# DLR-RM/AugmentedAutoencoder

Hardware: NVIDIA H100
Metric: pose queries/sec (encode+codebook NN) (higher is better)
Workload: dtype f32 via split-fp16 tensor-core products (3x, fp32 accumulate)

## Files before the change

### augmentedautoencoder_b200/csrc/tc_common.cuh

```cuda
#pragma once
#include <cuda.h>
#include <cuda_fp16.h>
#include <cuda_runtime.h>
#include <stdint.h>

namespace aae {
namespace tc {

__device__ __forceinline__ uint32_t smem_u32(const void* p) { return (uint32_t)__cvta_generic_to_shared(p); }

__device__ __forceinline__ bool elect_one() {
  uint32_t pred = 0;
  asm volatile(
      "{\n\t"
      ".reg .pred P1;\n\t"
      "elect.sync _|P1, 0xffffffff;\n\t"
      "selp.b32 %0, 1, 0, P1;\n\t"
      "}\n"
      : "=r"(pred));
  return pred != 0;
}

__device__ __forceinline__ void mbar_init(uint64_t* bar, uint32_t count) {
  asm volatile("mbarrier.init.shared::cta.b64 [%0], %1;" ::"r"(smem_u32(bar)), "r"(count));
}
__device__ __forceinline__ void fence_barrier_init() { asm volatile("fence.mbarrier_init.release.cluster;" ::: "memory"); }
__device__ __forceinline__ void fence_proxy_async_smem() { asm volatile("fence.proxy.async.shared::cta;" ::: "memory"); }

__device__ __forceinline__ void mbar_arrive_expect_tx(uint64_t* bar, uint32_t bytes) {
  asm volatile("mbarrier.arrive.expect_tx.shared::cta.b64 _, [%0], %1;" ::"r"(smem_u32(bar)), "r"(bytes) : "memory");
}
__device__ __forceinline__ void mbar_arrive(uint64_t* bar) {
  asm volatile("mbarrier.arrive.shared::cta.b64 _, [%0];" ::"r"(smem_u32(bar)) : "memory");
}
__device__ __forceinline__ bool mbar_try_wait(uint64_t* bar, uint32_t parity) {
  uint32_t ok;
  asm volatile(
      "{\n\t"
      ".reg .pred P1;\n\t"
      "mbarrier.try_wait.parity.shared::cta.b64 P1, [%1], %2;\n\t"
      "selp.b32 %0, 1, 0, P1;\n\t"
      "}\n"
      : "=r"(ok)
      : "r"(smem_u32(bar)), "r"(parity)
      : "memory");
  return ok != 0;
}
__device__ __forceinline__ void mbar_wait(uint64_t* bar, uint32_t parity) {
  while (!mbar_try_wait(bar, parity)) {
  }
}

__device__ __forceinline__ void prefetch_tmap(const CUtensorMap* m) {
  asm volatile("prefetch.tensormap [%0];" ::"l"(reinterpret_cast<uint64_t>(m)) : "memory");
}
__device__ __forceinline__ void tma_load_2d(void* smem_dst, const CUtensorMap* m, uint64_t* bar, int c0, int c1) {
  asm volatile("cp.async.bulk.tensor.2d.shared::cluster.global.mbarrier::complete_tx::bytes [%0], [%1, {%3, %4}], [%2];" ::"r"(
                   smem_u32(smem_dst)),
               "l"(reinterpret_cast<uint64_t>(m)), "r"(smem_u32(bar)), "r"(c0), "r"(c1)
               : "memory");
}
__device__ __forceinline__ void tma_load_4d(void* smem_dst, const CUtensorMap* m, uint64_t* bar, int c0, int c1, int c2, int c3) {
  asm volatile(
      "cp.async.bulk.tensor.4d.shared::cluster.global.mbarrier::complete_tx::bytes [%0], [%1, {%3, %4, %5, %6}], [%2];" ::"r"(
          smem_u32(smem_dst)),
      "l"(reinterpret_cast<uint64_t>(m)), "r"(smem_u32(bar)), "r"(c0), "r"(c1), "r"(c2), "r"(c3)
      : "memory");
}

__device__ __forceinline__ void bulk_store_1d(void* gmem_dst, const void* smem_src, uint32_t bytes) {
  asm volatile("cp.async.bulk.global.shared::cta.bulk_group [%0], [%1], %2;" ::"l"(gmem_dst), "r"(smem_u32(smem_src)), "r"(bytes) : "memory");
}
__device__ __forceinline__ void bulk_commit_group() { asm volatile("cp.async.bulk.commit_group;" ::: "memory"); }
__device__ __forceinline__ void bulk_wait_read_all() { asm volatile("cp.async.bulk.wait_group.read 0;" ::: "memory"); }
__device__ __forceinline__ void bulk_wait_all() { asm volatile("cp.async.bulk.wait_group 0;" ::: "memory"); }
__device__ __forceinline__ void tma_store_2d(const CUtensorMap* m, const void* smem_src, int c0, int c1) {
  asm volatile("cp.async.bulk.tensor.2d.global.shared::cta.bulk_group [%0, {%2, %3}], [%1];" ::"l"(reinterpret_cast<uint64_t>(m)),
               "r"(smem_u32(smem_src)), "r"(c0), "r"(c1)
               : "memory");
}
__device__ __forceinline__ void tma_store_5d(const CUtensorMap* m, const void* smem_src, int c0, int c1, int c2, int c3, int c4) {
  asm volatile("cp.async.bulk.tensor.5d.global.shared::cta.bulk_group [%0, {%2, %3, %4, %5, %6}], [%1];" ::"l"(reinterpret_cast<uint64_t>(m)),
               "r"(smem_u32(smem_src)), "r"(c0), "r"(c1), "r"(c2), "r"(c3), "r"(c4)
               : "memory");
}

template <int N>
struct Wgmma;
#define AAE_D8(i) "+f"(d[i]), "+f"(d[i + 1]), "+f"(d[i + 2]), "+f"(d[i + 3]), "+f"(d[i + 4]), "+f"(d[i + 5]), "+f"(d[i + 6]), "+f"(d[i + 7])
template <>
struct Wgmma<64> {
  template <int TA, int TB>
  static __device__ __forceinline__ void ss(float (&d)[32], uint64_t da, uint64_t db, uint32_t accumulate) {
    asm volatile(
        "{\n\t.reg .pred p;\n\tsetp.ne.b32 p, %34, 0;\n\t"
        "wgmma.mma_async.sync.aligned.m64n64k16.f32.f16.f16 {%0, %1, %2, %3, %4, %5, %6, %7, %8, %9, %10, %11, %12, %13, %14, %15, %16, %17, %18, %19, %20, %21, %22, %23, %24, %25, %26, %27, %28, %29, %30, %31}, %32, %33, p, 1, 1, %35, %36;\n\t}\n"
        : AAE_D8(0), AAE_D8(8), AAE_D8(16), AAE_D8(24)
        : "l"(da), "l"(db), "r"(accumulate), "n"(TA), "n"(TB));
  }
};

template <>
struct Wgmma<128> {
  template <int TA, int TB>
  static __device__ __forceinline__ void ss(float (&d)[64], uint64_t da, uint64_t db, uint32_t accumulate) {
    asm volatile(
        "{\n\t.reg .pred p;\n\tsetp.ne.b32 p, %66, 0;\n\t"
        "wgmma.mma_async.sync.aligned.m64n128k16.f32.f16.f16 {%0, %1, %2, %3, %4, %5, %6, %7, %8, %9, %10, %11, %12, %13, %14, %15, %16, %17, %18, %19, %20, %21, %22, %23, %24, %25, %26, %27, %28, %29, %30, %31, %32, %33, %34, %35, %36, %37, %38, %39, %40, %41, %42, %43, %44, %45, %46, %47, %48, %49, %50, %51, %52, %53, %54, %55, %56, %57, %58, %59, %60, %61, %62, %63}, %64, %65, p, 1, 1, %67, %68;\n\t}\n"
        : AAE_D8(0), AAE_D8(8), AAE_D8(16), AAE_D8(24), AAE_D8(32), AAE_D8(40), AAE_D8(48), AAE_D8(56)
        : "l"(da), "l"(db), "r"(accumulate), "n"(TA), "n"(TB));
  }
};

__device__ __forceinline__ void wgmma_fence() { asm volatile("wgmma.fence.sync.aligned;" ::: "memory"); }
__device__ __forceinline__ void wgmma_commit() { asm volatile("wgmma.commit_group.sync.aligned;" ::: "memory"); }
template <int N>
__device__ __forceinline__ void wgmma_wait() { asm volatile("wgmma.wait_group.sync.aligned %0;" ::"n"(N) : "memory"); }
template <int R>
__device__ __forceinline__ void wgmma_fence_regs(float (&d)[R]) {
#pragma unroll
  for (int i = 0; i < R; ++i) asm volatile("" : "+f"(d[i])::"memory");
}

__device__ __forceinline__ void cp_async_16(void* smem_dst, const void* gmem_src, bool pred) {
  const int bytes = pred ? 16 : 0;
  asm volatile("cp.async.cg.shared.global [%0], [%1], 16, %2;" ::"r"(smem_u32(smem_dst)), "l"(gmem_src), "r"(bytes) : "memory");
}
__device__ __forceinline__ void cp_async_wait_all() { asm volatile("cp.async.wait_all;" ::: "memory"); }
__device__ __forceinline__ void named_bar_sync(int id, int threads) { asm volatile("bar.sync %0, %1;" ::"r"(id), "r"(threads) : "memory"); }

__device__ __forceinline__ uint64_t make_sw128_kmajor_desc(uint32_t smem_addr) {
  uint64_t d = 0;
  d |= (uint64_t)((smem_addr & 0x3FFFF) >> 4);
  d |= (uint64_t)1 << 16;
  d |= (uint64_t)(1024 >> 4) << 32;
  d |= (uint64_t)1 << 62;
  return d;
}
__device__ __forceinline__ uint64_t make_sw128_mnmajor_desc(uint32_t smem_addr, uint32_t lbo_bytes, uint32_t sbo_bytes) {
  uint64_t d = 0;
  d |= (uint64_t)((smem_addr & 0x3FFFF) >> 4);
  d |= (uint64_t)(lbo_bytes >> 4) << 16;
  d |= (uint64_t)(sbo_bytes >> 4) << 32;
  d |= (uint64_t)1 << 62;
  return d;
}
__device__ __forceinline__ uint64_t desc_advance_k(uint64_t desc, int k_step) { return desc + (uint64_t)((k_step * 32) >> 4); }

__device__ __forceinline__ void split_f16(float x, __half& hi, __half& lo) {
  hi = __float2half_rn(x);
  lo = __float2half_rn(x - __half2float(hi));
}

__device__ __forceinline__ void split_f16x2(float a, float b, uint32_t& hi2, uint32_t& lo2) {
  const float ca = __fmul_rn(a, 8193.0f), cb = __fmul_rn(b, 8193.0f);
  const float ha = __fsub_rn(ca, __fsub_rn(ca, a)), hb = __fsub_rn(cb, __fsub_rn(cb, b));
  const __half2 h = __floats2half2_rn(ha, hb);
  const __half2 l = __floats2half2_rn(__fsub_rn(a, ha), __fsub_rn(b, hb));
  hi2 = *reinterpret_cast<const uint32_t*>(&h);
  lo2 = *reinterpret_cast<const uint32_t*>(&l);
}

}

typedef CUresult (*PFN_tmapEncodeTiled)(CUtensorMap*, CUtensorMapDataType, cuuint32_t, void*, const cuuint64_t*, const cuuint64_t*,
                                        const cuuint32_t*, const cuuint32_t*, CUtensorMapInterleave, CUtensorMapSwizzle,
                                        CUtensorMapL2promotion, CUtensorMapFloatOOBfill);
PFN_tmapEncodeTiled get_tmap_encoder();
int make_tmap_f16(CUtensorMap* out, const void* base, int rank, const uint64_t* dims, const uint64_t* strides_bytes, const uint32_t* box,
                  int swizzle_bytes = 128);

}
```

### augmentedautoencoder_b200/csrc/tc_gemm.cu

```cuda
#include <algorithm>
#include <vector>

#include "tc.cuh"
#include "tc_common.cuh"
#include "tc_plan.cuh"

namespace aae {

using namespace tc;

PFN_tmapEncodeTiled get_tmap_encoder() {
  static PFN_tmapEncodeTiled fn = nullptr;
  if (!fn) {
    void* p = nullptr;
    cudaDriverEntryPointQueryResult q;
    if (cudaGetDriverEntryPoint("cuTensorMapEncodeTiled", &p, cudaEnableDefault, &q) == cudaSuccess && q == cudaDriverEntryPointSuccess)
      fn = reinterpret_cast<PFN_tmapEncodeTiled>(p);
  }
  return fn;
}

int make_tmap_f16(CUtensorMap* out, const void* base, int rank, const uint64_t* dims, const uint64_t* strides_bytes, const uint32_t* box,
                  int swizzle_bytes) {
  PFN_tmapEncodeTiled enc = get_tmap_encoder();
  if (!enc) { set_error("cuTensorMapEncodeTiled is unavailable in this driver"); return AAE_ERR_CUDA; }
  cuuint64_t gdim[5], gstr[4];
  cuuint32_t bx[5], es[5];
  for (int i = 0; i < rank; ++i) { gdim[i] = dims[i]; bx[i] = box[i]; es[i] = 1; }
  for (int i = 0; i + 1 < rank; ++i) gstr[i] = strides_bytes[i];
  CUresult r = enc(out, CU_TENSOR_MAP_DATA_TYPE_FLOAT16, (cuuint32_t)rank, const_cast<void*>(base), gdim, gstr, bx, es,
                   CU_TENSOR_MAP_INTERLEAVE_NONE, swizzle_bytes == 64 ? CU_TENSOR_MAP_SWIZZLE_64B : CU_TENSOR_MAP_SWIZZLE_128B,
                   CU_TENSOR_MAP_L2_PROMOTION_L2_256B,
                   CU_TENSOR_MAP_FLOAT_OOB_FILL_NONE);
  if (r != CUDA_SUCCESS) { set_error("cuTensorMapEncodeTiled failed with CUresult %d (rank %d)", (int)r, rank); return AAE_ERR_CUDA; }
  return AAE_OK;
}

template <int N_TILE, int STAGES, int PLANES = 2>
struct TcSmem {
  static constexpr int A_BYTES = 128 * TC_KCH * 2;
  static constexpr int W_BYTES = N_TILE * TC_KCH * 2;
  static constexpr int STAGE_BYTES = PLANES * A_BYTES + PLANES * W_BYTES;
  static constexpr int ACC_LD = PLANES * N_TILE + 4;
  static constexpr int ACC_BYTES = 128 * ACC_LD * 4;
  static constexpr int BODY = STAGES * STAGE_BYTES > ACC_BYTES ? STAGES * STAGE_BYTES : ACC_BYTES;
  static constexpr int TOTAL = BODY + 1024  + 256 ;
};

template <int N_TILE, int STAGES, int PLANES = 2>
__global__ void __launch_bounds__(TC_THREADS, 1)
tc_gemm_kernel(const __grid_constant__ CUtensorMap tm_a_hi, const __grid_constant__ CUtensorMap tm_a_lo,
               const __grid_constant__ CUtensorMap tm_w_hi, const __grid_constant__ CUtensorMap tm_w_lo, const TcGemmParams p) {
  using S = TcSmem<N_TILE, STAGES, PLANES>;
  constexpr int R = N_TILE / 2;
  extern __shared__ uint8_t smem_raw[];
  uint8_t* smem = reinterpret_cast<uint8_t*>((reinterpret_cast<uintptr_t>(smem_raw) + 1023) & ~(uintptr_t)1023);
  uint64_t* full_bar = reinterpret_cast<uint64_t*>(smem + S::BODY);
  uint64_t* empty_bar = full_bar + STAGES;

  const int warp = threadIdx.x >> 5;
  const int lane = threadIdx.x & 31;
  const int m0 = blockIdx.y * 128;
  const int n0 = blockIdx.x * N_TILE;
  const int total_iters = p.taps * p.chunks_per_tap;
  const int it_begin = blockIdx.z * p.iters_per_split;
  const int it_end = min(total_iters, it_begin + p.iters_per_split);

  if (threadIdx.x == 0) {
    prefetch_tmap(&tm_a_hi);
    if constexpr (PLANES == 2) prefetch_tmap(&tm_a_lo);
    prefetch_tmap(&tm_w_hi);
    if constexpr (PLANES == 2) prefetch_tmap(&tm_w_lo);
    for (int s = 0; s < STAGES; ++s) { mbar_init(&full_bar[s], 1); mbar_init(&empty_bar[s], 2); }
    fence_barrier_init();
  }
  __syncthreads();

  if (warp == 0) {
    if (lane == 0) {
      const int hw = p.OH * p.OW;
      const int b0 = m0 / hw, rem = m0 - b0 * hw;
      const int oh0 = rem / p.OW, ow0 = rem - oh0 * p.OW;
      for (int it = it_begin, i = 0; it < it_end; ++it, ++i) {
        const int s = i % STAGES;
        const uint32_t ph = (uint32_t)(i / STAGES) & 1u;
        mbar_wait(&empty_bar[s], ph ^ 1u);
        const int tap = it / p.chunks_per_tap, cc = it - tap * p.chunks_per_tap;
        uint8_t* st = smem + s * S::STAGE_BYTES;
        mbar_arrive_expect_tx(&full_bar[s], S::STAGE_BYTES);
        const int c0 = p.tap_ch[tap] + cc * TC_KCH;
        const int x = ow0 + p.tap_dj[tap], y = oh0 + p.tap_di[tap];
        const int kcol = it * TC_KCH;
        tma_load_4d(st, &tm_a_hi, &full_bar[s], c0, x, y, b0);
        if constexpr (PLANES == 2) tma_load_4d(st + S::A_BYTES, &tm_a_lo, &full_bar[s], c0, x, y, b0);
        tma_load_2d(st + PLANES * S::A_BYTES, &tm_w_hi, &full_bar[s], kcol, n0);
        if constexpr (PLANES == 2) tma_load_2d(st + 2 * S::A_BYTES + S::W_BYTES, &tm_w_lo, &full_bar[s], kcol, n0);
      }
    }
  } else if (warp >= 4) {
    const int wg = (warp - 4) >> 2;
    float acc[R], crs[R];
#pragma unroll
    for (int j = 0; j < R; ++j) { acc[j] = 0.f; crs[j] = 0.f; }
    for (int it = it_begin, i = 0; it < it_end; ++it, ++i) {
      const int s = i % STAGES;
      mbar_wait(&full_bar[s], (uint32_t)(i / STAGES) & 1u);
      const uint32_t st = smem_u32(smem + s * S::STAGE_BYTES);
      const uint32_t a_off = (uint32_t)(wg * 64 * TC_KCH * 2);
      const uint64_t a_hi = make_sw128_kmajor_desc(st + a_off);
      const uint64_t a_lo = make_sw128_kmajor_desc(st + S::A_BYTES + a_off);
      const uint64_t w_hi = make_sw128_kmajor_desc(st + PLANES * S::A_BYTES);
      const uint64_t w_lo = make_sw128_kmajor_desc(st + 2 * S::A_BYTES + S::W_BYTES);
      wgmma_fence_regs(acc);
      if constexpr (PLANES == 2) wgmma_fence_regs(crs);
      wgmma_fence();
#pragma unroll
      for (int k = 0; k < TC_KCH / 16; ++k) {
        const uint32_t first = (i > 0 || k > 0) ? 1u : 0u;
        Wgmma<N_TILE>::template ss<0, 0>(acc, desc_advance_k(a_hi, k), desc_advance_k(w_hi, k), first);
        if constexpr (PLANES == 2) {
          Wgmma<N_TILE>::template ss<0, 0>(crs, desc_advance_k(a_lo, k), desc_advance_k(w_hi, k), first);
          Wgmma<N_TILE>::template ss<0, 0>(crs, desc_advance_k(a_hi, k), desc_advance_k(w_lo, k), 1u);
        }
      }
      wgmma_commit();
      wgmma_wait<1>();
      wgmma_fence_regs(acc);
      if constexpr (PLANES == 2) wgmma_fence_regs(crs);
      if (i > 0 && (warp & 3) == 0 && lane == 0) mbar_arrive(&empty_bar[(i - 1) % STAGES]);
    }
    wgmma_wait<0>();
    wgmma_fence_regs(acc);
    if constexpr (PLANES == 2) wgmma_fence_regs(crs);
    named_bar_sync(1, 256);
    float* img = reinterpret_cast<float*>(smem);
    tc_park_acc<PLANES>(img, S::ACC_LD, wg, warp, lane, acc, crs);
    named_bar_sync(1, 256);
    tc_epilogue<PLANES, N_TILE>(p, img, S::ACC_LD, m0, n0, it_end > it_begin, warp, lane);
  }
}

namespace {

template <int PLANES>
__global__ void pack_weights_kernel(const float* __restrict__ w, int taps, int cin, int cout, float scale, __half* __restrict__ hi,
                                    __half* __restrict__ lo, unsigned* __restrict__ range_flag, unsigned range_bit) {
  __shared__ float tile[32][33];
  const int tap = blockIdx.z;
  const int ci0 = blockIdx.y * 32, co0 = blockIdx.x * 32;
  for (int i = threadIdx.y; i < 32; i += 8) {
    const int ci = ci0 + i, co = co0 + threadIdx.x;
    tile[i][threadIdx.x] = (ci < cin && co < cout) ? w[((long long)tap * cin + ci) * cout + co] : 0.f;
  }
  __syncthreads();
  for (int i = threadIdx.y; i < 32; i += 8) {
    const int co = co0 + i, ci = ci0 + threadIdx.x;
    if (co < cout && ci < cin)
      tc_store_f16<PLANES>(tile[threadIdx.x][i] * scale, hi, lo, (long long)co * taps * cin + (long long)tap * cin + ci, range_flag, range_bit);
  }
}

template <int PLANES>
__global__ void unpack_act_kernel(const __half* __restrict__ hi, const __half* __restrict__ lo, int B, int H, int W, int C, int s2d,
                                  float inv_scale, float* __restrict__ out) {
  const long long total = (long long)B * H * W * C;
  for (long long i = (long long)blockIdx.x * blockDim.x + threadIdx.x; i < total; i += (long long)gridDim.x * blockDim.x) {
    const int c = (int)(i % C);
    long long r = i / C;
    const int w = (int)(r % W); r /= W;
    const int h = (int)(r % H);
    const int b = (int)(r / H);
    long long src = i;
    if (s2d) src = ((long long)(b * (H >> 1) + (h >> 1)) * (W >> 1) + (w >> 1)) * (4LL * C) + (((h & 1) << 1) | (w & 1)) * C + c;
    out[i] = tc_load_f16<PLANES>(hi, lo, src) * inv_scale;
  }
}

}

namespace {

template <int PLANES>
__global__ void __launch_bounds__(256) splitk_forward_finish_kernel(const float* __restrict__ partials, int splits, const TcGemmParams p) {
  const long long groups = (long long)p.M * (p.N >> 3);
  for (long long gi = (long long)blockIdx.x * blockDim.x + threadIdx.x; gi < groups; gi += (long long)gridDim.x * blockDim.x) {
    const int m = (int)(gi / (p.N >> 3)), n = (int)(gi - (long long)m * (p.N >> 3)) << 3;
    float f[8] = {0.f, 0.f, 0.f, 0.f, 0.f, 0.f, 0.f, 0.f};
    const float* src = partials + (long long)m * p.N + n;
    for (int sp = 0; sp < splits; ++sp, src += (long long)p.M * p.N) {
      const float4 a = *reinterpret_cast<const float4*>(src), b = *reinterpret_cast<const float4*>(src + 4);
      f[0] += a.x; f[1] += a.y; f[2] += a.z; f[3] += a.w; f[4] += b.x; f[5] += b.y; f[6] += b.z; f[7] += b.w;
    }
    float amax = 0.f;
#pragma unroll
    for (int j = 0; j < 8; ++j) {
      float v = f[j] + (p.bias ? __ldg(p.bias + n + j) : 0.f);
      if (p.relu == 1) v = fmaxf(v, 0.f);
      amax = fmaxf(amax, fabsf(v));
      f[j] = v * p.out_scale;
    }
    if (p.range_flag != nullptr && !(amax * p.out_scale < TC_F16_OVERFLOW)) atomicOr(p.range_flag, p.range_bit);
    tc_store_f16<PLANES>(f, 1.f, p.out_hi, p.out_lo, tc_decode_row(p, m).row_off + n);
  }
}

int dev_alloc(void** p, size_t bytes) { return tc_dev_alloc(p, bytes); }

bool pow2(int v) { return v > 0 && (v & (v - 1)) == 0; }

}

int tc_dev_alloc(void** p, size_t bytes) {
  cudaError_t e = cudaMalloc(p, bytes);
  if (e != cudaSuccess) { *p = nullptr; set_error("cudaMalloc(%zu) failed: %s", bytes, cudaGetErrorString(e)); return AAE_ERR_OOM; }
  cudaMemset(*p, 0, bytes);
  return AAE_OK;
}

int TcPlanes::alloc(size_t n, int planes) {
  AAE_TRY(tc_dev_alloc((void**)&hi, n * sizeof(__half)));
  return planes == 2 ? tc_dev_alloc((void**)&lo, n * sizeof(__half)) : AAE_OK;
}

void TcPlanes::release() {
  cudaFree(hi);
  cudaFree(lo);
  hi = lo = nullptr;
}

int TcPlanes::encode(TcMaps& m, int rank, const uint64_t* dims, const uint64_t* strides_bytes, const uint32_t* box, int swizzle_bytes) const {
  AAE_TRY(make_tmap_f16(&m.hi, hi, rank, dims, strides_bytes, box, swizzle_bytes));
  if (lo == nullptr) {
    m.lo = m.hi;
    return AAE_OK;
  }
  return make_tmap_f16(&m.lo, lo, rank, dims, strides_bytes, box, swizzle_bytes);
}

constexpr int TC_STAGES_SPLIT = 3, TC_STAGES_FP16 = 6;
static_assert(TcSmem<TC_N_TILE, TC_STAGES_FP16, 1>::TOTAL == TcSmem<TC_N_TILE, TC_STAGES_SPLIT>::TOTAL, "same footprint");

int tc_launch_layer(const TcLayer& T, dim3 tiles, cudaStream_t s, int planes) {
  AAE_REQUIRE(tiles.x <= 65535u, "tc_gemm: %u row tiles exceed the grid's y limit", tiles.x);
  return with_planes(planes, [&](auto P) {
    constexpr int STAGES = P == 1 ? TC_STAGES_FP16 : TC_STAGES_SPLIT;
    using S = TcSmem<TC_N_TILE, STAGES, P>;
    auto kern = tc_gemm_kernel<TC_N_TILE, STAGES, P>;
    AAE_CUDA_OK(cudaFuncSetAttribute(kern, cudaFuncAttributeMaxDynamicSharedMemorySize, S::TOTAL));
    kern<<<dim3(tiles.y, tiles.x, tiles.z), TC_THREADS, S::TOTAL, s>>>(T.tm_a.hi, T.tm_a.lo, T.tm_w.hi, T.tm_w.lo, T.gp);
    AAE_LAUNCH_OK();
    return AAE_OK;
  });
}

int tc_encoder_create(int device, const aae_net_cfg* cfg, TcEncoder** out) {
  *out = nullptr;
  const int L = cfg->num_layers;
  AAE_REQUIRE(aae_device_supported(device), "AAE_PREC_TC_SPLIT needs a compute-capability 9.0 device (wgmma/TMA)");
  AAE_REQUIRE(L >= 2, "AAE_PREC_TC_SPLIT: at least two conv layers expected");
  const int planes = tc_planes(cfg->precision);
  if (planes == 1 && !tc_conv1_supported(cfg)) {
    set_error("AAE_PREC_TC_FP16: the first layer needs the tensor-core conv1 (128 x 128 x 3 crops, 128 filters, k = 5, stride 2)");
    return AAE_ERR_UNSUPPORTED;
  }
  TcEncoder* h = new TcEncoder();
  h->device = device;
  h->cfg = *cfg;
  h->planes = planes;
  int ih = (cfg->in_h + cfg->strides[0] - 1) / cfg->strides[0], iw = (cfg->in_w + cfg->strides[0] - 1) / cfg->strides[0], ic = cfg->filters[0];
  const int B = cfg->max_batch;
  int st = AAE_OK;
  for (int l = 1; l <= L && st == AAE_OK; ++l) {
    TcLayer T;
    memset(&T.gp, 0, sizeof(T.gp));
    const bool dense = (l == L);
    if (!dense) {
      if (cfg->strides[l] != 2 || cfg->kernel_size != 5 || (ih & 1) || (iw & 1) || ic % 64 != 0 || cfg->filters[l] % 32 != 0) {
        set_error("AAE_PREC_TC_SPLIT: layer %d unsupported (needs k=5, stride 2, even dims, Cin %% 64 == 0, Cout %% 32 == 0)", l);
        st = AAE_ERR_UNSUPPORTED;
        break;
      }
      T.in_h = ih; T.in_w = iw; T.in_c = ic;
      T.out_h = ih / 2; T.out_w = iw / 2; T.out_c = cfg->filters[l];
      T.taps = 25;
      if (!pow2(T.out_w) || !pow2(T.out_h) || T.out_w > 128) { set_error("AAE_PREC_TC_SPLIT: output dims must be powers of two <= 128"); st = AAE_ERR_UNSUPPORTED; break; }
      T.BW = T.out_w;
      T.BH = std::min(T.out_h, 128 / T.BW);
      T.BB = 128 / (T.BW * T.BH);
    } else {
      T.in_h = T.in_w = 1; T.in_c = ih * iw * ic;
      T.out_h = T.out_w = 1; T.out_c = cfg->latent;
      T.taps = 1; T.BW = 1; T.BH = 1; T.BB = 128;
      h->flat = T.in_c;
      if (T.in_c % 64 != 0 || T.out_c % 32 != 0) { set_error("AAE_PREC_TC_SPLIT: dense layer needs flat %% 64 == 0 and latent %% 32 == 0"); st = AAE_ERR_UNSUPPORTED; break; }
    }
    const int B_pad = (int)ceil_div(B, T.BB) * T.BB;
    if ((st = T.in.alloc((size_t)B_pad * T.in_h * T.in_w * T.in_c, planes)) != AAE_OK) break;
    if ((st = T.w.alloc((size_t)T.out_c * T.taps * T.in_c, planes)) != AAE_OK) break;
    if (!dense) {
      const uint64_t C4 = 4ull * T.in_c, W2 = T.in_w / 2, H2 = T.in_h / 2;
      const uint64_t dims[4] = {C4, W2, H2, (uint64_t)B_pad};
      const uint64_t strides[3] = {C4 * 2, W2 * C4 * 2, H2 * W2 * C4 * 2};
      const uint32_t box[4] = {(uint32_t)TC_KCH, (uint32_t)T.BW, (uint32_t)T.BH, (uint32_t)T.BB};
      if ((st = T.in.encode(T.tm_a, 4, dims, strides, box)) != AAE_OK) break;
    } else {
      const uint64_t dims[4] = {(uint64_t)T.in_c, 1, 1, (uint64_t)B_pad};
      const uint64_t strides[3] = {(uint64_t)T.in_c * 2, (uint64_t)T.in_c * 2, (uint64_t)T.in_c * 2};
      const uint32_t box[4] = {(uint32_t)TC_KCH, 1, 1, 128};
      if ((st = T.in.encode(T.tm_a, 4, dims, strides, box)) != AAE_OK) break;
    }
    {
      const uint64_t K = (uint64_t)T.taps * T.in_c;
      const uint64_t dims[2] = {K, (uint64_t)T.out_c};
      const uint64_t strides[1] = {K * 2};
      const uint32_t box[2] = {(uint32_t)TC_KCH, (uint32_t)std::min(TC_N_TILE, T.out_c)};
      if ((st = T.w.encode(T.tm_w, 2, dims, strides, box)) != AAE_OK) break;
    }
    TcGemmParams& g = T.gp;
    g.N = T.out_c; g.OH = T.out_h; g.OW = T.out_w; g.BW = T.BW; g.BH = T.BH;
    g.taps = T.taps; g.chunks_per_tap = T.in_c / TC_KCH;
    g.iters_per_split = g.taps * g.chunks_per_tap;
    for (int t = 0; t < T.taps; ++t) {
      if (dense) { g.tap_di[t] = 0; g.tap_dj[t] = 0; g.tap_ch[t] = 0; continue; }
      const int kh = t / 5, kw = t % 5;
      g.tap_di[t] = (int8_t)((kh + 1) / 2 - 1);
      g.tap_dj[t] = (int8_t)((kw + 1) / 2 - 1);
      g.tap_ch[t] = ((((kh + 1) & 1) << 1) | ((kw + 1) & 1)) * T.in_c;
    }
    g.unscale = 1.f / (ACT_SCALE * W_SCALE);
    g.out_scale = ACT_SCALE;
    g.relu = dense ? 0 : 1;
    h->layers.push_back(T);
    if (!dense) { ih = T.out_h; iw = T.out_w; ic = T.out_c; }
  }
  if (st == AAE_OK) {
    for (size_t i = 0; i + 1 < h->layers.size(); ++i) {
      TcGemmParams& g = h->layers[i].gp;
      g.out_hi = h->layers[i + 1].in.hi;
      g.out_lo = h->layers[i + 1].in.lo;
      g.out_mode = (i + 2 == h->layers.size()) ? OUT_PLAIN_SPLIT : OUT_S2D_SPLIT;
    }
    TcLayer& D = h->layers.back();
    const int total = D.gp.taps * D.gp.chunks_per_tap;
    h->dense_splits = std::min(total, 66);
    D.gp.iters_per_split = (total + h->dense_splits - 1) / h->dense_splits;
    h->dense_splits = (total + D.gp.iters_per_split - 1) / D.gp.iters_per_split;
    D.gp.out_mode = OUT_F32;
    st = dev_alloc((void**)&h->partials, (size_t)h->dense_splits * (B + 128) * cfg->latent * sizeof(float));
    D.gp.out_f32 = h->partials;
  }
  if (st == AAE_OK) st = dev_alloc((void**)&h->range_flag, sizeof(unsigned));
  if (st == AAE_OK)
    for (size_t i = 0; i + 1 < h->layers.size(); ++i) {
      h->layers[i].gp.range_flag = h->range_flag;
      h->layers[i].gp.range_bit = 1u << (i + 1);
    }
  if (st == AAE_OK && tc_conv1_supported(cfg)) st = tc_conv1_create(device, cfg, &h->conv1);
  if (st != AAE_OK) { tc_encoder_destroy(h); return st; }
  *out = h;
  return AAE_OK;
}

void tc_encoder_destroy(TcEncoder* h) {
  if (!h) return;
  for (auto& T : h->layers) { T.in.release(); T.w.release(); }
  cudaFree(h->partials);
  cudaFree(h->fwd_partials);
  cudaFree(h->dbg);
  if (h->owns_range_flag) cudaFree(h->range_flag);
  tc_conv1_destroy(h->conv1);
  delete h;
}

int tc_encoder_pack_weights(TcEncoder* h, int layer, const float* w_dev, cudaStream_t s) {
  if (layer == 0) {
    if (h->conv1) return tc_conv1_pack(h->conv1, w_dev, h->cfg.kernel_size * h->cfg.kernel_size * h->cfg.in_c, W_SCALE, h->range_flag, 1u << 16, s);
    return AAE_OK;
  }
  AAE_REQUIRE(layer >= 1 && layer <= (int)h->layers.size(), "tc pack: layer %d out of range", layer);
  TcLayer& T = h->layers[layer - 1];
  dim3 grid((unsigned)ceil_div(T.out_c, 32), (unsigned)ceil_div(T.in_c, 32), (unsigned)T.taps), block(32, 8);
  with_planes(h->planes, [&](auto P) {
    pack_weights_kernel<P><<<grid, block, 0, s>>>(w_dev, T.taps, T.in_c, T.out_c, W_SCALE, T.w.hi, T.w.lo, h->range_flag, 1u << (16 + layer));
  });
  AAE_LAUNCH_OK();
  return AAE_OK;
}

unsigned* tc_encoder_range_flag(TcEncoder* h) { return h->range_flag; }
unsigned* tc_decoder_range_flag(TcDecoder* h) { return h->range_flag; }

void tc_encoder_share_range_flag(TcEncoder* h, unsigned* flag) {
  if (h->owns_range_flag) cudaFree(h->range_flag);
  h->range_flag = flag;
  h->owns_range_flag = false;
  for (size_t i = 0; i + 1 < h->layers.size(); ++i) h->layers[i].gp.range_flag = flag;
}

void tc_decoder_share_range_flag(TcDecoder* h, unsigned* flag) {
  if (h->owns_range_flag) cudaFree(h->range_flag);
  h->range_flag = flag;
  h->owns_range_flag = false;
// ... 327 lines not shown
```

### augmentedautoencoder_b200/csrc/tc_plan.cuh

```cuda
#pragma once
#include <stdlib.h>

#include <type_traits>
#include <vector>

#include "tc.cuh"
#include "tc_common.cuh"

namespace aae {

enum TcOutMode : int {
  OUT_S2D_SPLIT = 0,
  OUT_PLAIN_SPLIT = 1,
  OUT_F32 = 2,
  OUT_D2S_SPLIT = 3
};

struct TcGemmParams {
  int M;
  int N;
  int OH, OW;
  int BW, BH;
  int taps;
  int chunks_per_tap;
  int iters_per_split;
  int8_t tap_di[32], tap_dj[32];
  int tap_ch[32];
  float unscale;
  const unsigned* amax_bits;
  float out_scale;
  const float* bias;
  int relu;
  int out_mode;
  __half* out_hi;
  __half* out_lo;
  float* out_f32;
  unsigned* range_flag;
  unsigned range_bit;
};

constexpr float TC_F16_OVERFLOW = 65520.f;



__host__ __device__ __forceinline__ int tc_dyn_exponent(unsigned amax_bits) {
  int e = (int)((amax_bits >> 23) & 0xffu) - 127;
  return e < -100 ? -100 : (e > 100 ? 100 : e);
}
__device__ __forceinline__ float tc_dyn_scale(unsigned amax_bits) { return __int_as_float((127 + 13 - tc_dyn_exponent(amax_bits)) << 23); }
__device__ __forceinline__ float tc_dyn_unscale(unsigned amax_bits) { return __int_as_float((127 - 13 + tc_dyn_exponent(amax_bits)) << 23); }

constexpr float ACT_SCALE = 16.f;
constexpr float W_SCALE = 256.f;
constexpr int TC_STAGES = 2;
constexpr int TC_THREADS = 384;
constexpr int TC_N_TILE = 128;
constexpr int TC_KCH = 64;

struct TcMaps {
  CUtensorMap hi, lo;
};

struct TcPlanes {
  __half* hi = nullptr;
  __half* lo = nullptr;
  int alloc(size_t n, int planes);
  void release();
  int encode(TcMaps& m, int rank, const uint64_t* dims, const uint64_t* strides_bytes, const uint32_t* box, int swizzle_bytes = 128) const;
};

template <class F>
auto with_planes(int planes, F&& f) {
  return planes == 1 ? f(std::integral_constant<int, 1>{}) : f(std::integral_constant<int, 2>{});
}

struct TcLayer {
  int in_h, in_w, in_c, out_h, out_w, out_c;
  int taps, BW, BH, BB;
  TcPlanes in;
  TcPlanes w;
  TcMaps tm_a, tm_w;
  TcGemmParams gp;
};

struct TcEncoder {
  int device;
  aae_net_cfg cfg;
  unsigned* range_flag = nullptr;
  bool owns_range_flag = true;
  std::vector<TcLayer> layers;
  int flat;
  float* partials = nullptr;
  float* fwd_partials = nullptr;
  size_t fwd_partial_floats = 0;
  int dense_splits = 1;
  TcConv1* conv1 = nullptr;
  int planes = 2;
  float* dbg = nullptr;
  size_t dbg_floats = 0;
};


struct TcDecoder {
  int device;
  aae_net_cfg cfg;
  unsigned* range_flag = nullptr;
  bool owns_range_flag = true;
  std::vector<TcLayer> layers;
  std::vector<float*> bias_dev;
  float* wm_tmp = nullptr;
  float* out_p = nullptr;
  const float* out_bias = nullptr;
  size_t wm_floats = 0;
  int planes = 2;
};


struct TcRow {
  bool valid;
  int b, i, j;
  long long row_off;
};

__device__ __forceinline__ TcRow tc_decode_row(const TcGemmParams& p, int m) {
  TcRow r;
  r.valid = m < p.M;
  r.b = r.i = r.j = 0;
  r.row_off = 0;
  if (!r.valid) return r;
  const int hw = p.OH * p.OW;
  r.b = m / hw;
  const int rem = m - r.b * hw;
  r.i = rem / p.OW;
  r.j = rem - r.i * p.OW;
  if (p.out_mode == OUT_S2D_SPLIT)
    r.row_off = ((long long)(r.b * (p.OH >> 1) + (r.i >> 1)) * (p.OW >> 1) + (r.j >> 1)) * (4LL * p.N) + (((r.i & 1) << 1) | (r.j & 1)) * p.N;
  else
    r.row_off = (long long)m * p.N;
  return r;
}


template <int PLANES, int N>
__device__ __forceinline__ void tc_store_f16(const float (&v)[N], float scale, __half* hi, __half* lo, long long off,
                                             unsigned* range_flag = nullptr, unsigned range_bit = 0) {
  uint32_t h[N / 2], l[N / 2];
  float amax = 0.f;
#pragma unroll
  for (int j = 0; j < N; j += 2) {
    amax = fmaxf(amax, fmaxf(fabsf(v[j]), fabsf(v[j + 1])));
    if constexpr (PLANES == 1) {
      const __half2 p = __floats2half2_rn(v[j] * scale, v[j + 1] * scale);
      h[j >> 1] = *reinterpret_cast<const uint32_t*>(&p);
    } else {
      tc::split_f16x2(v[j] * scale, v[j + 1] * scale, h[j >> 1], l[j >> 1]);
    }
  }
  if (range_flag != nullptr && !(amax * scale < TC_F16_OVERFLOW)) atomicOr(range_flag, range_bit);
  if constexpr (N == 2) {
    *reinterpret_cast<uint32_t*>(hi + off) = h[0];
    if constexpr (PLANES == 2) *reinterpret_cast<uint32_t*>(lo + off) = l[0];
  } else if constexpr (N == 4) {
    *reinterpret_cast<uint2*>(hi + off) = make_uint2(h[0], h[1]);
    if constexpr (PLANES == 2) *reinterpret_cast<uint2*>(lo + off) = make_uint2(l[0], l[1]);
  } else {
#pragma unroll
    for (int j = 0; j < N / 8; ++j) {
      reinterpret_cast<uint4*>(hi + off)[j] = make_uint4(h[4 * j], h[4 * j + 1], h[4 * j + 2], h[4 * j + 3]);
      if constexpr (PLANES == 2) reinterpret_cast<uint4*>(lo + off)[j] = make_uint4(l[4 * j], l[4 * j + 1], l[4 * j + 2], l[4 * j + 3]);
    }
  }
}

template <int PLANES>
__device__ __forceinline__ void tc_store_f16(float v, __half* hi, __half* lo, long long i, unsigned* range_flag = nullptr,
                                             unsigned range_bit = 0) {
  if (range_flag != nullptr && !(fabsf(v) < TC_F16_OVERFLOW)) atomicOr(range_flag, range_bit);
  __half h, l;
  tc::split_f16(v, h, l);
  hi[i] = h;
  if constexpr (PLANES == 2) lo[i] = l;
}

template <int PLANES>
__device__ __forceinline__ float tc_load_f16(const __half* hi, const __half* lo, long long i) {
  if constexpr (PLANES == 1) return __half2float(hi[i]);
  else return __half2float(hi[i]) + __half2float(lo[i]);
}

template <int PLANES>
__device__ __forceinline__ void tc_store_chunk(const TcGemmParams& p, const TcRow& r, int n, float (&f)[32], int split_z) {
  if (p.out_mode == OUT_F32) {
    float* dst = p.out_f32 + (long long)split_z * p.M * p.N + r.row_off + n;
#pragma unroll
    for (int j = 0; j < 32; j += 4) *reinterpret_cast<float4*>(dst + j) = make_float4(f[j], f[j + 1], f[j + 2], f[j + 3]);
    return;
  }
  float b[32];
  if (p.bias != nullptr) {
#pragma unroll
    for (int j = 0; j < 32; ++j) b[j] = __ldg(p.bias + n + j);
  } else {
#pragma unroll
    for (int j = 0; j < 32; ++j) b[j] = 0.f;
  }
  const float floor_v = p.relu == 1 ? 0.f : -INFINITY;
#pragma unroll
  for (int j = 0; j < 32; ++j) f[j] = fmaxf(f[j] + b[j], floor_v);
  long long off = r.row_off + n;
  if (p.out_mode == OUT_D2S_SPLIT) {
    const int cq = p.N >> 2, cls = n / cq, co = n - cls * cq;
    off = ((long long)(r.b * 2 * p.OH + 2 * r.i + (cls >> 1)) * (2 * p.OW) + 2 * r.j + (cls & 1)) * cq + co;
  }
  tc_store_f16<PLANES>(f, p.out_scale, p.out_hi, p.out_lo, off, p.range_flag, p.range_bit);
}


template <int PLANES, int R>
__device__ __forceinline__ void tc_park_acc(float* img, int ld, int wg, int warp, int lane, const float (&acc)[R], const float (&crs)[R]) {
  const int r0 = wg * 64 + (warp & 3) * 16 + (lane >> 2), c0 = (lane & 3) * 2;
#pragma unroll
  for (int j = 0; j < R / 4; ++j) {
    *reinterpret_cast<float2*>(img + r0 * ld + 8 * j + c0) = make_float2(acc[4 * j], acc[4 * j + 1]);
    *reinterpret_cast<float2*>(img + (r0 + 8) * ld + 8 * j + c0) = make_float2(acc[4 * j + 2], acc[4 * j + 3]);
    if constexpr (PLANES == 2) {
      *reinterpret_cast<float2*>(img + r0 * ld + 2 * R + 8 * j + c0) = make_float2(crs[4 * j], crs[4 * j + 1]);
      *reinterpret_cast<float2*>(img + (r0 + 8) * ld + 2 * R + 8 * j + c0) = make_float2(crs[4 * j + 2], crs[4 * j + 3]);
    }
  }
}
__device__ __forceinline__ void tc_acc_ld32(const float* img, int ld, int row, int col, uint32_t (&v)[32]) {
  const float4* src = reinterpret_cast<const float4*>(img + row * ld + col);
#pragma unroll
  for (int j = 0; j < 8; ++j) {
    const float4 f = src[j];
    v[4 * j] = __float_as_uint(f.x); v[4 * j + 1] = __float_as_uint(f.y); v[4 * j + 2] = __float_as_uint(f.z); v[4 * j + 3] = __float_as_uint(f.w);
  }
}

template <int PLANES, int N_TILE>
__device__ __forceinline__ void tc_epilogue(const TcGemmParams& p, const float* img, int ld, int m0, int n0, bool has_work, int warp, int lane) {
  const int q = warp & 3, half = (warp - 4) >> 2;
  const TcRow row = tc_decode_row(p, m0 + q * 32 + lane);
  const float unscale = p.amax_bits ? p.unscale * tc_dyn_unscale(__ldg(p.amax_bits)) : p.unscale;
#pragma unroll 1
  for (int c = half; c < N_TILE / 32; c += 2) {
    const int n = n0 + c * 32;
    if (!row.valid || n >= p.N) continue;
    uint32_t v[32], x[32];
    tc_acc_ld32(img, ld, q * 32 + lane, c * 32, v);
    if constexpr (PLANES == 2) tc_acc_ld32(img, ld, q * 32 + lane, N_TILE + c * 32, x);
    float f[32];
#pragma unroll
    for (int j = 0; j < 32; ++j) {
      if constexpr (PLANES == 1) f[j] = has_work ? __uint_as_float(v[j]) * unscale : 0.f;
      else f[j] = has_work ? (__uint_as_float(v[j]) + __uint_as_float(x[j])) * unscale : 0.f;
    }
    tc_store_chunk<PLANES>(p, row, n, f, (int)blockIdx.z);
  }
}

int tc_launch_layer(const TcLayer& T, dim3 grid, cudaStream_t s, int planes);
int tc_dev_alloc(void** p, size_t bytes);
int tc_layer_setup_plain(TcLayer& T, int B, int planes);

}
```

Measured before the change: 35770.

## Make tensor-core GEMM persistent with register-direct epilogue overlapped with next tile

Converts the split-fp16 GEMM kernel to a persistent grid of at most SM-count CTAs that loop over tiles, keeping the TMA/mbarrier pipeline running across tile boundaries. The epilogue now writes from accumulator fragments in registers, in two halves interleaved with the next tile's first wgmma iterations, instead of parking the accumulators in shared memory behind named barriers. Producer and consumer warpgroups rebalance registers with setmaxnreg to make room for the extra value buffer. This aims to hide epilogue and launch-tail cost, at the price of narrower float2 global stores, higher register pressure, and changes to the tc_store_f16 call signature and range-flag reporting.

New measurement: 37970, median of 6. +6.1%, better.

```diff
diff --git a/augmentedautoencoder_b200/csrc/tc_common.cuh b/augmentedautoencoder_b200/csrc/tc_common.cuh
--- a/augmentedautoencoder_b200/csrc/tc_common.cuh
+++ b/augmentedautoencoder_b200/csrc/tc_common.cuh
@@ -122,6 +122,11 @@
   for (int i = 0; i < R; ++i) asm volatile("" : "+f"(d[i])::"memory");
 }
 
+template <int N>
+__device__ __forceinline__ void setmaxnreg_dec() { asm volatile("setmaxnreg.dec.sync.aligned.u32 %0;" ::"n"(N)); }
+template <int N>
+__device__ __forceinline__ void setmaxnreg_inc() { asm volatile("setmaxnreg.inc.sync.aligned.u32 %0;" ::"n"(N)); }
+
 __device__ __forceinline__ void cp_async_16(void* smem_dst, const void* gmem_src, bool pred) {
   const int bytes = pred ? 16 : 0;
   asm volatile("cp.async.cg.shared.global [%0], [%1], 16, %2;" ::"r"(smem_u32(smem_dst)), "l"(gmem_src), "r"(bytes) : "memory");
diff --git a/augmentedautoencoder_b200/csrc/tc_gemm.cu b/augmentedautoencoder_b200/csrc/tc_gemm.cu
--- a/augmentedautoencoder_b200/csrc/tc_gemm.cu
+++ b/augmentedautoencoder_b200/csrc/tc_gemm.cu
@@ -1,3 +1,5 @@
+#include <limits.h>
+
 #include <algorithm>
 #include <vector>
 
@@ -41,16 +43,31 @@
   static constexpr int A_BYTES = 128 * TC_KCH * 2;
   static constexpr int W_BYTES = N_TILE * TC_KCH * 2;
   static constexpr int STAGE_BYTES = PLANES * A_BYTES + PLANES * W_BYTES;
-  static constexpr int ACC_LD = PLANES * N_TILE + 4;
-  static constexpr int ACC_BYTES = 128 * ACC_LD * 4;
-  static constexpr int BODY = STAGES * STAGE_BYTES > ACC_BYTES ? STAGES * STAGE_BYTES : ACC_BYTES;
+  static constexpr int BODY = STAGES * STAGE_BYTES;
   static constexpr int TOTAL = BODY + 1024  + 256 ;
 };
+
+struct TcTile {
+  int m0, n0, z, it_begin, it_end;
+};
+template <int N_TILE>
+__device__ __forceinline__ TcTile tc_tile(const TcGemmParams& p, const TcTiles& g, int t) {
+  TcTile r;
+  const int yz = t / g.n;
+  const int y = yz % g.m;
+  r.z = yz / g.m;
+  r.m0 = y * 128;
+  r.n0 = (t - yz * g.n) * N_TILE;
+  r.it_begin = r.z * p.iters_per_split;
+  r.it_end = min(p.taps * p.chunks_per_tap, r.it_begin + p.iters_per_split);
+  return r;
+}
 
 template <int N_TILE, int STAGES, int PLANES = 2>
 __global__ void __launch_bounds__(TC_THREADS, 1)
 tc_gemm_kernel(const __grid_constant__ CUtensorMap tm_a_hi, const __grid_constant__ CUtensorMap tm_a_lo,
-               const __grid_constant__ CUtensorMap tm_w_hi, const __grid_constant__ CUtensorMap tm_w_lo, const TcGemmParams p) {
+               const __grid_constant__ CUtensorMap tm_w_hi, const __grid_constant__ CUtensorMap tm_w_lo, const TcGemmParams p,
+               const TcTiles tiles) {
   using S = TcSmem<N_TILE, STAGES, PLANES>;
   constexpr int R = N_TILE / 2;
   extern __shared__ uint8_t smem_raw[];
@@ -60,11 +77,6 @@
 
   const int warp = threadIdx.x >> 5;
   const int lane = threadIdx.x & 31;
-  const int m0 = blockIdx.y * 128;
-  const int n0 = blockIdx.x * N_TILE;
-  const int total_iters = p.taps * p.chunks_per_tap;
-  const int it_begin = blockIdx.z * p.iters_per_split;
-  const int it_end = min(total_iters, it_begin + p.iters_per_split);
 
   if (threadIdx.x == 0) {
     prefetch_tmap(&tm_a_hi);
@@ -76,67 +88,85 @@
   }
   __syncthreads();
 
-  if (warp == 0) {
-    if (lane == 0) {
+  if (warp < 4) {
+    setmaxnreg_dec<TC_PRODUCER_REGS>();
+    if (warp == 0 && lane == 0) {
       const int hw = p.OH * p.OW;
-      const int b0 = m0 / hw, rem = m0 - b0 * hw;
-      const int oh0 = rem / p.OW, ow0 = rem - oh0 * p.OW;
-      for (int it = it_begin, i = 0; it < it_end; ++it, ++i) {
+      int i = 0;
+      for (int t = blockIdx.x; t < tiles.count; t += gridDim.x) {
+        const TcTile T = tc_tile<N_TILE>(p, tiles, t);
+        const int b0 = T.m0 / hw, rem = T.m0 - b0 * hw;
+        const int oh0 = rem / p.OW, ow0 = rem - oh0 * p.OW;
+        for (int it = T.it_begin; it < T.it_end; ++it, ++i) {
+          const int s = i % STAGES;
+          const uint32_t ph = (uint32_t)(i / STAGES) & 1u;
+          mbar_wait(&empty_bar[s], ph ^ 1u);
+          const int tap = it / p.chunks_per_tap, cc = it - tap * p.chunks_per_tap;
+          uint8_t* st = smem + s * S::STAGE_BYTES;
+          mbar_arrive_expect_tx(&full_bar[s], S::STAGE_BYTES);
+          const int c0 = p.tap_ch[tap] + cc * TC_KCH;
+          const int x = ow0 + p.tap_dj[tap], y = oh0 + p.tap_di[tap];
+          const int kcol = it * TC_KCH;
+          tma_load_4d(st, &tm_a_hi, &full_bar[s], c0, x, y, b0);
+          if constexpr (PLANES == 2) tma_load_4d(st + S::A_BYTES, &tm_a_lo, &full_bar[s], c0, x, y, b0);
+          tma_load_2d(st + PLANES * S::A_BYTES, &tm_w_hi, &full_bar[s], kcol, T.n0);
+          if constexpr (PLANES == 2) tma_load_2d(st + 2 * S::A_BYTES + S::W_BYTES, &tm_w_lo, &full_bar[s], kcol, T.n0);
+        }
+      }
+    }
+  } else {
+    setmaxnreg_inc<TC_CONSUMER_REGS>();
+    const int wg = (warp - 4) >> 2;
+    const bool releases = (warp & 3) == 0 && lane == 0;
+    constexpr int H = R / 8;
+    float acc[R], crs[R], v[R];
+#pragma unroll
+    for (int j = 0; j < R; ++j) { acc[j] = 0.f; crs[j] = 0.f; v[j] = 0.f; }
+    int pm0 = 0, pn0 = 0, pz = 0, half = 2;
+    auto epilogue_half = [&](int h) {
+      if (h == 0) tc_epilogue_frag<PLANES, 0, H>(p, v, pm0, pn0, pz, warp, lane);
+      else tc_epilogue_frag<PLANES, H, 2 * H>(p, v, pm0, pn0, pz, warp, lane);
+    };
+    int i = 0;
+    for (int t = blockIdx.x; t < tiles.count; t += gridDim.x) {
+      const TcTile T = tc_tile<N_TILE>(p, tiles, t);
+      for (int it = T.it_begin; it < T.it_end; ++it, ++i) {
         const int s = i % STAGES;
-        const uint32_t ph = (uint32_t)(i / STAGES) & 1u;
-        mbar_wait(&empty_bar[s], ph ^ 1u);
-        const int tap = it / p.chunks_per_tap, cc = it - tap * p.chunks_per_tap;
-        uint8_t* st = smem + s * S::STAGE_BYTES;
-        mbar_arrive_expect_tx(&full_bar[s], S::STAGE_BYTES);
-        const int c0 = p.tap_ch[tap] + cc * TC_KCH;
-        const int x = ow0 + p.tap_dj[tap], y = oh0 + p.tap_di[tap];
-        const int kcol = it * TC_KCH;
-        tma_load_4d(st, &tm_a_hi, &full_bar[s], c0, x, y, b0);
-        if constexpr (PLANES == 2) tma_load_4d(st + S::A_BYTES, &tm_a_lo, &full_bar[s], c0, x, y, b0);
-        tma_load_2d(st + PLANES * S::A_BYTES, &tm_w_hi, &full_bar[s], kcol, n0);
-        if constexpr (PLANES == 2) tma_load_2d(st + 2 * S::A_BYTES + S::W_BYTES, &tm_w_lo, &full_bar[s], kcol, n0);
+        mbar_wait(&full_bar[s], (uint32_t)(i / STAGES) & 1u);
+        const uint32_t st = smem_u32(smem + s * S::STAGE_BYTES);
+        const uint32_t a_off = (uint32_t)(wg * 64 * TC_KCH * 2);
+        const uint64_t a_hi = make_sw128_kmajor_desc(st + a_off);
+        const uint64_t a_lo = make_sw128_kmajor_desc(st + S::A_BYTES + a_off);
+        const uint64_t w_hi = make_sw128_kmajor_desc(st + PLANES * S::A_BYTES);
+        const uint64_t w_lo = make_sw128_kmajor_desc(st + 2 * S::A_BYTES + S::W_BYTES);
+        wgmma_fence_regs(acc);
+        if constexpr (PLANES == 2) wgmma_fence_regs(crs);
+        wgmma_fence();
+#pragma unroll
+        for (int k = 0; k < TC_KCH / 16; ++k) {
+          const uint32_t first = (it > T.it_begin || k > 0) ? 1u : 0u;
+          Wgmma<N_TILE>::template ss<0, 0>(acc, desc_advance_k(a_hi, k), desc_advance_k(w_hi, k), first);
+          if constexpr (PLANES == 2) {
+            Wgmma<N_TILE>::template ss<0, 0>(crs, desc_advance_k(a_lo, k), desc_advance_k(w_hi, k), first);
+            Wgmma<N_TILE>::template ss<0, 0>(crs, desc_advance_k(a_hi, k), desc_advance_k(w_lo, k), 1u);
+          }
+        }
+        wgmma_commit();
+        if (half < 2) epilogue_half(half++);
+        wgmma_wait<1>();
+        wgmma_fence_regs(acc);
+        if constexpr (PLANES == 2) wgmma_fence_regs(crs);
+        if (it > T.it_begin && releases) mbar_arrive(&empty_bar[(i - 1) % STAGES]);
       }
-    }
-  } else if (warp >= 4) {
-    const int wg = (warp - 4) >> 2;
-    float acc[R], crs[R];
-#pragma unroll
-    for (int j = 0; j < R; ++j) { acc[j] = 0.f; crs[j] = 0.f; }
-    for (int it = it_begin, i = 0; it < it_end; ++it, ++i) {
-      const int s = i % STAGES;
-      mbar_wait(&full_bar[s], (uint32_t)(i / STAGES) & 1u);
-      const uint32_t st = smem_u32(smem + s * S::STAGE_BYTES);
-      const uint32_t a_off = (uint32_t)(wg * 64 * TC_KCH * 2);
-      const uint64_t a_hi = make_sw128_kmajor_desc(st + a_off);
-      const uint64_t a_lo = make_sw128_kmajor_desc(st + S::A_BYTES + a_off);
-      const uint64_t w_hi = make_sw128_kmajor_desc(st + PLANES * S::A_BYTES);
-      const uint64_t w_lo = make_sw128_kmajor_desc(st + 2 * S::A_BYTES + S::W_BYTES);
+      wgmma_wait<0>();
       wgmma_fence_regs(acc);
       if constexpr (PLANES == 2) wgmma_fence_regs(crs);
-      wgmma_fence();
-#pragma unroll
-      for (int k = 0; k < TC_KCH / 16; ++k) {
-        const uint32_t first = (i > 0 || k > 0) ? 1u : 0u;
-        Wgmma<N_TILE>::template ss<0, 0>(acc, desc_advance_k(a_hi, k), desc_advance_k(w_hi, k), first);
-        if constexpr (PLANES == 2) {
-          Wgmma<N_TILE>::template ss<0, 0>(crs, desc_advance_k(a_lo, k), desc_advance_k(w_hi, k), first);
-          Wgmma<N_TILE>::template ss<0, 0>(crs, desc_advance_k(a_hi, k), desc_advance_k(w_lo, k), 1u);
-        }
-      }
-      wgmma_commit();
-      wgmma_wait<1>();
-      wgmma_fence_regs(acc);
-      if constexpr (PLANES == 2) wgmma_fence_regs(crs);
-      if (i > 0 && (warp & 3) == 0 && lane == 0) mbar_arrive(&empty_bar[(i - 1) % STAGES]);
-    }
-    wgmma_wait<0>();
-    wgmma_fence_regs(acc);
-    if constexpr (PLANES == 2) wgmma_fence_regs(crs);
-    named_bar_sync(1, 256);
-    float* img = reinterpret_cast<float*>(smem);
-    tc_park_acc<PLANES>(img, S::ACC_LD, wg, warp, lane, acc, crs);
-    named_bar_sync(1, 256);
-    tc_epilogue<PLANES, N_TILE>(p, img, S::ACC_LD, m0, n0, it_end > it_begin, warp, lane);
+      if (T.it_end > T.it_begin && releases) mbar_arrive(&empty_bar[(i - 1) % STAGES]);
+      while (half < 2) epilogue_half(half++);
+      tc_epilogue_values<PLANES>(p, acc, crs, T.it_end > T.it_begin, v);
+      pm0 = T.m0 + wg * 64; pn0 = T.n0; pz = T.z; half = 0;
+    }
+    while (half < 2) epilogue_half(half++);
   }
 }
 
@@ -241,13 +271,19 @@
 static_assert(TcSmem<TC_N_TILE, TC_STAGES_FP16, 1>::TOTAL == TcSmem<TC_N_TILE, TC_STAGES_SPLIT>::TOTAL, "same footprint");
 
 int tc_launch_layer(const TcLayer& T, dim3 tiles, cudaStream_t s, int planes) {
-  AAE_REQUIRE(tiles.x <= 65535u, "tc_gemm: %u row tiles exceed the grid's y limit", tiles.x);
+  const long long count = (long long)tiles.x * tiles.y * tiles.z;
+  AAE_REQUIRE(count <= INT_MAX, "tc_gemm: %lld tiles exceed the kernel's int tile index", count);
+  int device = 0, sms = 0;
+  AAE_CUDA_OK(cudaGetDevice(&device));
+  AAE_CUDA_OK(cudaDeviceGetAttribute(&sms, cudaDevAttrMultiProcessorCount, device));
+  const TcTiles g{(int)tiles.y, (int)tiles.x, (int)count};
+  const unsigned ctas = (unsigned)std::min<long long>(count, sms);
   return with_planes(planes, [&](auto P) {
     constexpr int STAGES = P == 1 ? TC_STAGES_FP16 : TC_STAGES_SPLIT;
     using S = TcSmem<TC_N_TILE, STAGES, P>;
     auto kern = tc_gemm_kernel<TC_N_TILE, STAGES, P>;
     AAE_CUDA_OK(cudaFuncSetAttribute(kern, cudaFuncAttributeMaxDynamicSharedMemorySize, S::TOTAL));
-    kern<<<dim3(tiles.y, tiles.x, tiles.z), TC_THREADS, S::TOTAL, s>>>(T.tm_a.hi, T.tm_a.lo, T.tm_w.hi, T.tm_w.lo, T.gp);
+    kern<<<ctas, TC_THREADS, S::TOTAL, s>>>(T.tm_a.hi, T.tm_a.lo, T.tm_w.hi, T.tm_w.lo, T.gp, g);
     AAE_LAUNCH_OK();
     return AAE_OK;
   });
diff --git a/augmentedautoencoder_b200/csrc/tc_plan.cuh b/augmentedautoencoder_b200/csrc/tc_plan.cuh
--- a/augmentedautoencoder_b200/csrc/tc_plan.cuh
+++ b/augmentedautoencoder_b200/csrc/tc_plan.cuh
@@ -55,6 +55,7 @@
 constexpr int TC_STAGES = 2;
 constexpr int TC_THREADS = 384;
 constexpr int TC_N_TILE = 128;
+constexpr int TC_PRODUCER_REGS = 24, TC_CONSUMER_REGS = 240;
 constexpr int TC_KCH = 64;
 
 struct TcMaps {
@@ -260,7 +261,62 @@
   }
 }
 
-int tc_launch_layer(const TcLayer& T, dim3 grid, cudaStream_t s, int planes);
+template <int PLANES, int R>
+__device__ __forceinline__ void tc_epilogue_values(const TcGemmParams& p, const float (&acc)[R], const float (&crs)[R], bool has_work,
+                                                   float (&v)[R]) {
+  const float unscale = p.amax_bits ? p.unscale * tc_dyn_unscale(__ldg(p.amax_bits)) : p.unscale;
+#pragma unroll
+  for (int e = 0; e < R; ++e) {
+    if constexpr (PLANES == 1) v[e] = has_work ? __fmul_rn(acc[e], unscale) : 0.f;
+    else v[e] = has_work ? __fmul_rn(__fadd_rn(acc[e], crs[e]), unscale) : 0.f;
+  }
+}
+
+template <int PLANES, int J0, int J1, int R>
+__device__ __forceinline__ void tc_epilogue_frag(const TcGemmParams& p, const float (&v)[R], int m0, int n0, int split_z, int warp, int lane) {
+  const int r0 = m0 + (warp & 3) * 16 + (lane >> 2), c0 = n0 + 2 * (lane & 3);
+  const TcRow rows[2] = {tc_decode_row(p, r0), tc_decode_row(p, r0 + 8)};
+  if (p.out_mode == OUT_F32) {
+    float* dst = p.out_f32 + (long long)split_z * p.M * p.N;
+#pragma unroll
+    for (int j = J0; j < J1; ++j) {
+      const int n = c0 + 8 * j;
+#pragma unroll
+      for (int h = 0; h < 2; ++h)
+        if (rows[h].valid && n < p.N) *reinterpret_cast<float2*>(dst + rows[h].row_off + n) = make_float2(v[4 * j + 2 * h], v[4 * j + 2 * h + 1]);
+    }
+    return;
+  }
+  const float floor_v = p.relu == 1 ? 0.f : -INFINITY;
+  const int cq = p.N >> 2;
+  float amax = 0.f;
+#pragma unroll
+  for (int j = J0; j < J1; ++j) {
+    const int n = c0 + 8 * j;
+    if (n >= p.N) continue;
+    const float b0 = p.bias != nullptr ? __ldg(p.bias + n) : 0.f, b1 = p.bias != nullptr ? __ldg(p.bias + n + 1) : 0.f;
+#pragma unroll
+    for (int h = 0; h < 2; ++h) {
+      const TcRow& r = rows[h];
+      if (!r.valid) continue;
+      float f[2] = {fmaxf(__fadd_rn(v[4 * j + 2 * h], b0), floor_v), fmaxf(__fadd_rn(v[4 * j + 2 * h + 1], b1), floor_v)};
+      amax = fmaxf(amax, fmaxf(fabsf(f[0]), fabsf(f[1])));
+      long long off = r.row_off + n;
+      if (p.out_mode == OUT_D2S_SPLIT) {
+        const int cls = n / cq, co = n - cls * cq;
+        off = ((long long)(r.b * 2 * p.OH + 2 * r.i + (cls >> 1)) * (2 * p.OW) + 2 * r.j + (cls & 1)) * cq + co;
+      }
+      tc_store_f16<PLANES>(f, p.out_scale, p.out_hi, p.out_lo, off);
+    }
+  }
+  if (p.range_flag != nullptr && !(amax * p.out_scale < TC_F16_OVERFLOW)) atomicOr(p.range_flag, p.range_bit);
+}
+
+struct TcTiles {
+  int n, m, count;
+};
+
+int tc_launch_layer(const TcLayer& T, dim3 tiles, cudaStream_t s, int planes);
 int tc_dev_alloc(void** p, size_t bytes);
 int tc_layer_setup_plain(TcLayer& T, int B, int planes);
 
```
